# vwxyzjn/cleanrl

Measured on NVIDIA H100. Metric: env steps/sec (SPS) PPO Breakout num_envs=1024, higher is better.
Workload: dtype bf16

## Files before the change

cleanrl_b200/csrc/net_tc.cu:

```cuda
#include <cuda.h>
#include <algorithm>
#include "tc_base.cuh"
#include "tc_conv_win.cuh"
#include "tc_conv1_u8.cuh"
#include "tc_gemm_tma.cuh"
#include "tc_wgrad_win.cuh"
#include "tc_reduce.cuh"
#include "tc_aux.cuh"
#include "tc_heads.cuh"
#include "tc_heads_wide.cuh"
#include "tc_lstm.cuh"

namespace b200rl {

struct NatureLayout {
    int A;
    int64_t c1w, c1b, c2w, c2b, c3w, c3b, fcw, fcb, hw, hb, total;
    int64_t w1f, w2f, w2dg, w3f, w3dg, wfcf, wfcdg, w1l, w1sc, packed_total;
    bool wide; int G; int64_t whf, whdg, hbp;
    int64_t wih, whh, bih, bhh, whhp;
    explicit NatureLayout(int A_) : A(A_), wih(-1), whh(-1), bih(-1), bhh(-1), whhp(-1) {
        int64_t o = 0;
        c1w = o; o += 32 * 4 * 8 * 8;  c1b = o; o += 32;
        c2w = o; o += 64 * 32 * 4 * 4; c2b = o; o += 64;
// ... 76 lines not shown
    }
};

static void gemm_rowmajor(KGemmParams& p, const bf16* x, int64_t n, int nchunks) {
    memset(&p, 0, sizeof(p));
    p.scale = 1.f;
    p.A = x; p.M = n; p.nchunks = nchunks;
}


static void win_defaults(WinParams& p) { memset(&p, 0, sizeof(p)); p.scale = 1.f; }
static int round8(int v) { return (v + 7) & ~7; }
static void win_conv1(WinParams& p, const bf16* x0, const int64_t* rows, int64_t n) {
    p.A = x0; p.rows = rows; p.n = (int)n; p.G = 441; p.Wp = 21; p.M = n * 441;
    p.tpi_shift = 2;
    p.n_images = rows ? (int64_t)1 << 24 : n;
    p.ntaps = 4; p.shift[0] = 0; p.shift[1] = 1; p.shift[2] = 21; p.shift[3] = 22; p.WR = round8(128 + 22);
}
static void win_conv2(WinParams& p, const bf16* act1, int64_t n) {
    p.A = act1; p.n = (int)n; p.G = 100; p.Wp = 10; p.M = n * 100;
    p.ntaps = 4; p.shift[0] = 0; p.shift[1] = 1; p.shift[2] = 10; p.shift[3] = 11; p.WR = round8(128 + 11);
}
static void win_conv3(WinParams& p, const bf16* act2, int64_t n) {
    p.A = act2; p.n = (int)n; p.G = 81; p.Wp = 9; p.M = n * 81;
    p.ntaps = 9; for (int ky = 0; ky < 3; ++ky) for (int kx = 0; kx < 3; ++kx) p.shift[ky * 3 + kx] = ky * 9 + kx;
    p.WR = round8(128 + 20);
}
static void wgw_defaults(WGradWinParams& w) { memset(&w, 0, sizeof(w)); }

static const int kC1Ctas = 264, kC2Ctas = 132, kC3Ctas = 132;
static WPlan conv1_wgrad_plan(int64_t n, bool u8) {
    return u8 ? wgrad_plan(n * 512, kC2Ctas, 512) : wgrad_plan(n * 512, kC1Ctas, 128);
}
static WPlan conv2_wgrad_plan(int64_t n) { return wgrad_plan(n * 100, kC2Ctas, 128); }
static WPlan conv3_wgrad_plan(int64_t n) { return wgrad_plan(n * 81, kC3Ctas, 128); }

static size_t wgrad_win_bytes(int splits, int nslots) { return (size_t)splits * nslots * 64 * 64 * sizeof(float); }
static size_t wgrad_win_bias_bytes(int splits) { return (size_t)splits * 64 * sizeof(float); }
static int launch_wgrad_win(const WGradWinParams& p, int ctas, cudaStream_t s, const char* what) {
    const size_t smem = (size_t)kWgradWinStages * ((size_t)p.WRX * 128 * p.cpr + 128 * 128) + 4096 + 1024;
    static SmemAttrCache attr;
    if (int rc0 = attr.ensure(tc_wgrad_win, smem, what)) return rc0;
    CUtensorMap tmX, tmY;
    memset(&tmX, 0, sizeof(tmX)); memset(&tmY, 0, sizeof(tmY));
    const int use_tma = p.tpi_shift ? 0 : 1;
    if (p.rows_per_cta % 128 != 0) return fail(B200RL_ERR_INVALID_ARGUMENT, "%s: rows per CTA must be a multiple of 128", what);
    if (ctas < 1 || (int64_t)(ctas - 1) * p.rows_per_cta >= p.M)
        return fail(B200RL_ERR_INVALID_ARGUMENT, "%s: every row split must own at least one row", what);
    int rc;
    if (use_tma) {
        if (p.rows || p.ldy != 64 || p.ncolsY != 64)
            return fail(B200RL_ERR_INVALID_ARGUMENT, "%s: linear-grid mode needs contiguous rows and 64-channel dY", what);
        if ((rc = make_tmap_2d(&tmX, p.X, p.M, (int64_t)p.cpr * 64, p.WRX, what))) return rc;
        if ((rc = make_tmap_2d(&tmY, p.Y, p.M, 64, 128, what))) return rc;
    } else {
        if ((128 << p.tpi_shift) < p.G) return fail(B200RL_ERR_INVALID_ARGUMENT, "%s: steps per image too small", what);
        if ((rc = make_tmap_3d(&tmX, p.X, p.n_images, p.G, (int64_t)p.cpr * 64, p.WRX, what))) return rc;
    }
    const dim3 grid((unsigned)ceil_div(p.nslots / 2, kWgradWinTilesPerCta), ctas);
    tc_wgrad_win<<<grid, kWgradWinThreads, smem, s>>>(tmX, tmY, p, use_tma);
    return check_launch(what);
}

}

using namespace b200rl;

namespace b200rl {
static bool head_ok(int A) { return A >= 1 && A < kMaxWideHeads; }
static size_t wide_dhead_bytes(int64_t n, const NatureLayout& L) { return ((size_t)n * L.G * 2 + 255) & ~(size_t)255; }
static size_t wide_small_bytes(int64_t n, const NatureLayout& L, int A1) {
    return wide_dhead_bytes(n, L) + colsum_f32_ws(n, A1);
}

static int trunk_fwd(const NatureLayout& L, const NatureActs& Q, const float* params, const bf16* P, bf16* act, int64_t n,
                     cudaStream_t s) {
    int rc;
    KGemmParams p;
    WinParams wp;
    win_defaults(wp); win_conv2(wp, act + Q.act1, n);
    wp.Bw = P + L.w2f; wp.N = 64; wp.vH = 9; wp.vW = 9; wp.out_mode = WOUT_DENSE; wp.out = act + Q.act2;
    wp.bias = params + L.c2b; wp.relu = 1; wp.mask_out = reinterpret_cast<uint32_t*>(act + Q.m2);
    { ProfScope ps(s, "conv2_fwd", 2.0 * n * 81 * 64 * 512, (double)n * ((12800 + 5184) * 2 + 648));
      if ((rc = launch_conv_win_t<128, 2, 2, 4>(wp, s, "naturecnn/conv2"))) return rc; }
    win_defaults(wp); win_conv3(wp, act + Q.act2, n);
    wp.Bw = P + L.w3f; wp.N = 64; wp.vH = 7; wp.vW = 7; wp.out_mode = WOUT_DENSE; wp.out = act + Q.act3;
    wp.bias = params + L.c3b; wp.relu = 1; wp.mask_out = reinterpret_cast<uint32_t*>(act + Q.m3);
    { ProfScope ps(s, "conv3_fwd", 2.0 * n * 49 * 64 * 576, (double)n * ((5184 + 3136) * 2 + 392));
      if ((rc = launch_conv_win_t<128, 1, 4, 9>(wp, s, "naturecnn/conv3"))) return rc; }
    gemm_rowmajor(p, act + Q.act3, n, 49);
    p.Bw = P + L.wfcf; p.N = 512; p.out = act + Q.hid; p.ldo = 512; p.bias = params + L.fcb; p.relu = 1;
    p.mask_out = reinterpret_cast<uint32_t*>(act + Q.m4);
    { ProfScope ps(s, "fc_fwd", 2.0 * n * 512 * 3136, (double)n * (3136 + 512) * 2 + 512.0 * 3136 * 2);
      if (n <= 8192) { if ((rc = launch_gemm_tma<64, 6>(p, s, "naturecnn/fc"))) return rc; }
      else if ((rc = launch_gemm_tma<128, 3>(p, s, "naturecnn/fc"))) return rc; }
    return B200RL_OK;
}

static int trunk_bwd(const NatureLayout& L, const NatureActs& Q, const bf16* P, bf16* act, float* grads, int64_t n,
                     float* wsbig, float* wssmall, void* tail_ready_event, bool dact1_fused, cudaStream_t s) {
    int rc;
    KGemmParams p;
    {
        int splits;
        { ProfScope ps(s, "fc_wgrad", 2.0 * n * 512 * 3136, (double)n * (3136 + 512) * 2 + 512.0 * 3136 * 4);
          if ((splits = launch_wgrad_tma(act + Q.dhid, 512, act + Q.act3, 3136, n, wsbig, s, "naturecnn/fc_wgrad")) < 0) return splits; }
        { ProfScope ps(s, "wgrad_fold_bias", 0, 0);
          note_launches(1); tc_fold_fc<<<(unsigned)ceil_div((int64_t)512 * 3136, 256), 256, 0, s>>>(wsbig, splits, 512, 13 * 256, 512, 3136, 64, 49, 1.f, grads + L.fcw);
          if ((rc = colsum(act + Q.dhid, n, 512, 512, wssmall, grads + L.fcb, s))) return rc; }
        if (tail_ready_event) {
            cudaError_t e = cudaEventRecord(reinterpret_cast<cudaEvent_t>(tail_ready_event), s);
            if (e != cudaSuccess) return fail(B200RL_ERR_CUDA, "naturecnn_backward: cudaEventRecord: %s", cudaGetErrorString(e));
        }
        gemm_rowmajor(p, act + Q.dhid, n, 8);
        p.Bw = P + L.wfcdg; p.N = 3136; p.out = act + Q.dact3a; p.out2 = act + Q.dact3b; p.dual_dact3 = 1;
        p.ldo = 3136; p.mask_bits = reinterpret_cast<const uint32_t*>(act + Q.m3);
        { ProfScope ps(s, "fc_dgrad", 2.0 * n * 512 * 3136, (double)n * ((3136 + 512) * 2 + 392) + 512.0 * 3136 * 2);
          if ((rc = launch_gemm_tma<128, 3>(p, s, "naturecnn/fc_dgrad"))) return rc; }
    }
    WGradWinParams gw;
    WinParams wp;
    FoldWin fw;
    {
        wgw_defaults(gw);
        gw.X = act + Q.act2; gw.M = n * 81; gw.n = (int)n; gw.G = 81; gw.cpr = 1; gw.nslots = 10; gw.WRX = round8(128 + 20);
        for (int t = 0; t < 9; ++t) gw.shift[t] = (t / 3) * 9 + (t % 3);
        const int st[10] = {0, 1, 2, 3, 4, 5, 6, 7, 7, 8};
        for (int k = 0; k < 10; ++k) { gw.slot_tap[k] = st[k]; gw.slot_cc[k] = 0; }
        gw.Y = act + Q.dact3a; gw.ldy = 64; gw.ncolsY = 64;
        const WPlan pl = conv3_wgrad_plan(n);
        gw.rows_per_cta = pl.rows_per_cta; gw.ws = wsbig; gw.wsb = wssmall;
        { ProfScope ps(s, "conv3_wgrad", 2.0 * n * 49 * 64 * 576, (double)n * (5184 + 5184) * 2);
          if ((rc = launch_wgrad_win(gw, pl.splits, s, "naturecnn/conv3_wgrad"))) return rc; }
        memset(&fw, 0, sizeof(fw));
        fw.layer = 3; fw.S = pl.splits; fw.nslots = 10; fw.Cout = 64; fw.scale = 1.f; fw.bscale = 1.f;
        for (int k = 0; k < 10; ++k) { fw.slot_tap[k] = st[k]; fw.slot_skip[k] = (k == 8); }
        { ProfScope ps(s, "wgrad_fold_bias", 0, 0);
          fw.wsb = wssmall; fw.db = grads + L.c3b;
          tc_fold_win<<<(unsigned)ceil_div(640 * 64 + 64, 32), 256, 0, s>>>(wsbig, fw, grads + L.c3w);
          if ((rc = check_launch("naturecnn/conv3_fold"))) return rc; }
        win_defaults(wp);
        wp.A = act + Q.dact3b; wp.n = (int)n; wp.G = 121; wp.Wp = 11; wp.M = n * 121; wp.ntaps = 9;
        for (int ky = 0; ky < 3; ++ky) for (int kx = 0; kx < 3; ++kx) wp.shift[ky * 3 + kx] = (2 - ky) * 11 + (2 - kx);
        wp.WR = round8(128 + 24);
        wp.Bw = P + L.w3dg; wp.N = 64; wp.vH = 9; wp.vW = 9; wp.out_mode = WOUT_DACT2;
        wp.out = act + Q.dact2a; wp.out2 = act + Q.dact2b; wp.mask_bits = reinterpret_cast<const uint32_t*>(act + Q.m2);
        { ProfScope ps(s, "conv3_dgrad", 2.0 * n * 81 * 64 * 576, (double)n * ((7744 + 6400 + 7744) * 2 + 648));
          if ((rc = launch_conv_win_t<128, 1, 4, 9>(wp, s, "naturecnn/conv3_dgrad"))) return rc; }
    }
    {
        wgw_defaults(gw);
        gw.X = act + Q.act1; gw.M = n * 100; gw.n = (int)n; gw.G = 100; gw.cpr = 2; gw.nslots = 8; gw.WRX = round8(128 + 11);
        gw.shift[0] = 0; gw.shift[1] = 1; gw.shift[2] = 10; gw.shift[3] = 11;
        for (int k = 0; k < 8; ++k) { gw.slot_tap[k] = k >> 1; gw.slot_cc[k] = k & 1; }
        gw.Y = act + Q.dact2a; gw.ldy = 64; gw.ncolsY = 64;
        const WPlan pl = conv2_wgrad_plan(n);
        gw.rows_per_cta = pl.rows_per_cta; gw.ws = wsbig; gw.wsb = wssmall;
        { ProfScope ps(s, "conv2_wgrad", 2.0 * n * 81 * 64 * 512, (double)n * (12800 + 6400) * 2);
          if ((rc = launch_wgrad_win(gw, pl.splits, s, "naturecnn/conv2_wgrad"))) return rc; }
        memset(&fw, 0, sizeof(fw));
        fw.layer = 2; fw.S = pl.splits; fw.nslots = 8; fw.Cout = 64; fw.scale = 1.f; fw.bscale = 1.f;
        for (int k = 0; k < 8; ++k) { fw.slot_tap[k] = k >> 1; fw.slot_cc[k] = k & 1; }
        { ProfScope ps(s, "wgrad_fold_bias", 0, 0);
          fw.wsb = wssmall; fw.db = grads + L.c2b;
          tc_fold_win<<<(unsigned)ceil_div(512 * 64 + 64, 32), 256, 0, s>>>(wsbig, fw, grads + L.c2w);
          if ((rc = check_launch("naturecnn/conv2_fold"))) return rc; }
        if (dact1_fused) return B200RL_OK;
        win_defaults(wp);
        wp.A = act + Q.dact2b; wp.n = (int)n; wp.G = 121; wp.Wp = 11; wp.M = n * 121; wp.ntaps = 4;
        for (int a = 0; a < 2; ++a) for (int b = 0; b < 2; ++b) wp.shift[a * 2 + b] = (1 - a) * 11 + (1 - b);
        wp.WR = round8(128 + 12);
        wp.Bw = P + L.w2dg; wp.N = 128; wp.vH = 10; wp.vW = 10; wp.out_mode = WOUT_DACT1;
        wp.out = act + Q.dact1; wp.mask_bits = reinterpret_cast<const uint32_t*>(act + Q.m1);
        { ProfScope ps(s, "conv2_dgrad", 2.0 * n * 400 * 32 * 256, (double)n * ((7744 + 14112) * 2 + 1600));
          if ((rc = launch_conv_win<128, 1, 4, 4>(wp, s, "naturecnn/conv2_dgrad"))) return rc; }
    }
    return B200RL_OK;
}
static size_t trunk_big_bytes(int64_t n) {
    return std::max({wgrad_tma_bytes(n, 512, 3136), wgrad_win_bytes(conv3_wgrad_plan(n).splits, 10),
                     wgrad_win_bytes(conv2_wgrad_plan(n).splits, 8)});
}
static size_t trunk_small_bytes(int64_t n) {
    return std::max({colsum_ws(n, 512), wgrad_win_bias_bytes(conv3_wgrad_plan(n).splits),
                     wgrad_win_bias_bytes(conv2_wgrad_plan(n).splits)});
}

static int wide_head_fwd(const NatureLayout& L, const bf16* P, const bf16* hid, int64_t n, int A1, float* out, cudaStream_t s) {
    KGemmParams p;
    gemm_rowmajor(p, hid, n, 8);
    p.Bw = P + L.whf; p.N = L.G; p.bias = reinterpret_cast<const float*>(P + L.hbp);
    p.out_f32 = out; p.ldo = A1; p.ncols_f32 = A1;
    return launch_gemm_tma<128, 3>(p, s, "wide_heads");
}

static int wide_head_bwd(const NatureLayout& L, const bf16* P, const float* dhead, int64_t n, int A1, const bf16* hid, bf16* dhid,
                         const uint32_t* hid_bits, float* dW, float* db, float* wsbig, float* wssmall, cudaStream_t s) {
    int rc;
    KGemmParams p;
    bf16* dh16 = reinterpret_cast<bf16*>(wssmall);
    float* dbpart = reinterpret_cast<float*>(reinterpret_cast<char*>(wssmall) + wide_dhead_bytes(n, L));
    int cb = (int)ceil_div(n * L.G, 256); if (cb > num_sms() * 8) cb = num_sms() * 8;
    tc_head_dhead_bf16<<<cb, 256, 0, s>>>(dhead, n, A1, L.G, dh16);
    if ((rc = check_launch("wide_heads_dhead"))) return rc;
    if ((rc = colsum_f32(dhead, n, A1, dbpart, db, s))) return rc;
    const int splits = launch_wgrad_tma(dh16, L.G, hid, 512, n, wsbig, s, "wide_heads_wgrad");
    if (splits < 0) return splits;
    tc_fold_fc<<<(unsigned)ceil_div((int64_t)A1 * 512, 256), 256, 0, s>>>(wsbig, splits, L.G, 512, A1, 512, 512, 1, 1.f, dW);
    if ((rc = check_launch("wide_heads_wgrad"))) return rc;
    gemm_rowmajor(p, dh16, n, L.G / 64);
    p.Bw = P + L.whdg; p.N = 512; p.out = dhid; p.ldo = 512;
    p.mask_bits = hid_bits;
    if (n <= 8192) { if ((rc = launch_gemm_tma<64, 6>(p, s, "wide_heads_dgrad"))) return rc; }
    else if ((rc = launch_gemm_tma<128, 3>(p, s, "wide_heads_dgrad"))) return rc;
    return B200RL_OK;
}
}

extern "C" int64_t b200rl_naturecnn_param_count(int A) { return A >= 1 ? NatureLayout(A).total : -1; }
extern "C" int64_t b200rl_naturecnn_grad_tail_offset(int A) { return A >= 1 ? NatureLayout(A).fcw : -1; }
extern "C" size_t b200rl_naturecnn_bf16_packed_bytes(int A) { return head_ok(A) ? (size_t)NatureLayout(A).packed_total * 2 : 0; }
extern "C" size_t b200rl_naturecnn_bf16_acts_bytes(int64_t n, int obs_format) {
    return n >= 0 ? (size_t)NatureActs(n, obs_format == B200RL_OBS_U8_NCHW).total * 2 + 256 : 0;
}

extern "C" int b200rl_frames_to_s2d_bf16(const uint8_t* obs, const int64_t* rows, int64_t n, void* out, void* stream) {
    B200RL_REQUIRE(n >= 0, "frames_to_s2d: negative n");
    if (n == 0) return B200RL_OK;
    B200RL_REQUIRE(obs && out, "frames_to_s2d: null pointer");
    B200RL_REQUIRE(aligned(obs, 4) && aligned(out, 16), "frames_to_s2d: misaligned buffer");
    cudaStream_t s = (cudaStream_t)stream;
// ... 373 lines not shown
```

cleanrl_b200/csrc/tc_conv_win.cuh:

```cuda
#pragma once
#include "tc_base.cuh"

namespace b200rl {
using namespace tc;

enum { WOUT_DENSE = 0, WOUT_S2D2 = 1, WOUT_DACT2 = 2, WOUT_DACT1 = 3 };
struct WinParams {
    const bf16* A;
    const int64_t* rows;
    int64_t M;
    int n, G, Wp;
    int tpi_shift;
    int64_t n_images;
    int ntaps;
    int shift[16];
    int WR;
    const bf16* Bw;
    int N;
    int vH, vW;
    int out_mode;
    bf16* out;
    bf16* out2;
    const uint32_t* mask_bits;
    uint32_t* mask_out;
// ... 168 lines not shown
                        const float f = __uint_as_float(v[e]);
                        bits |= (f > 0.f ? 1u : 0u) << e;
                    }
                    if (p.mask_out) p.mask_out[ob + g] = bits;
                }
                if (p.mask_bits) {
#pragma unroll
                    for (int e = 0; e < 32; ++e) if (!((mb[g] >> e) & 1u)) v[e] = 0u;
                }
                int4 w[4];
                if (p.relu) {
#pragma unroll
                    for (int e = 0; e < 4; ++e) {
                        w[e].x = (int)pack_bf16x2_relu(__uint_as_float(v[8 * e]), __uint_as_float(v[8 * e + 1]));
                        w[e].y = (int)pack_bf16x2_relu(__uint_as_float(v[8 * e + 2]), __uint_as_float(v[8 * e + 3]));
                        w[e].z = (int)pack_bf16x2_relu(__uint_as_float(v[8 * e + 4]), __uint_as_float(v[8 * e + 5]));
                        w[e].w = (int)pack_bf16x2_relu(__uint_as_float(v[8 * e + 6]), __uint_as_float(v[8 * e + 7]));
                    }
                } else {
#pragma unroll
                for (int e = 0; e < 4; ++e) {
                    w[e].x = (int)pack_bf16x2(__uint_as_float(v[8 * e]), __uint_as_float(v[8 * e + 1]));
                    w[e].y = (int)pack_bf16x2(__uint_as_float(v[8 * e + 2]), __uint_as_float(v[8 * e + 3]));
                    w[e].z = (int)pack_bf16x2(__uint_as_float(v[8 * e + 4]), __uint_as_float(v[8 * e + 5]));
                    w[e].w = (int)pack_bf16x2(__uint_as_float(v[8 * e + 6]), __uint_as_float(v[8 * e + 7]));
                }
                }
                if (p.out_mode == WOUT_DACT1) {
                    int4* brow = reinterpret_cast<int4*>(st + lr * LDA) + 8 * g + 4 * (g & 1);
#pragma unroll
                    for (int e = 0; e < 4; ++e) brow[e] = w[e];
                } else {
                    bf16* dst = p.out + o1 + g * 32;
                    st_global_32b(dst, w[0], w[1]);
                    st_global_32b(dst + 16, w[2], w[3]);
                }
            }
            if (p.out_mode == WOUT_DACT1) {
                if (half == 0)
                    *reinterpret_cast<int64_t*>(st + lr * LDA + BN) = valid ? ((int64_t)i * 441 + 2 * Y * 21 + 2 * X) * 32 : -1;
                named_bar(1 + wg, 128);
#pragma unroll
                for (int m = 0; m < 8; ++m) {
                    const int k = m * 128 + wt, g = (k >> 2) & 3, e = k & 3;
                    const float* srow = st + (k >> 4) * LDA;
                    const int64_t o = *reinterpret_cast<const int64_t*>(srow + BN);
                    if (o < 0) continue;
                    const int4 val = reinterpret_cast<const int4*>(srow)[8 * g + 4 * (g & 1) + e];
                    *reinterpret_cast<int4*>(p.out + o + (g >> 1) * 21 * 32 + (g & 1) * 32 + e * 8) = val;
                }
            }
        }
    }
}

template <int BN, int CPR, int STAGES, int NTAPS>
static int launch_conv_win(const WinParams& p, cudaStream_t s, const char* what) {
    if (p.ntaps != NTAPS) return fail(B200RL_ERR_INVALID_ARGUMENT, "%s: %d taps, kernel instance has %d", what, p.ntaps, NTAPS);
    if (p.out_mode != WOUT_S2D2 && p.out_mode != WOUT_DACT1)
        return fail(B200RL_ERR_INVALID_ARGUMENT, "%s: dense and conv3 data-gradient outputs run on tc_conv_win_t", what);
    if (p.out_mode == WOUT_DACT1 && (BN != 128 || p.N != 128))
        return fail(B200RL_ERR_INVALID_ARGUMENT, "%s: the conv2 data gradient stores 4 groups of 32 channels per cell", what);
    const size_t smem = (size_t)p.ntaps * CPR * BN * 128 + (size_t)STAGES * p.WR * 128 * CPR + conv_win_acc_bytes<BN>() + 1024;
    static SmemAttrCache attr;
    if (int rc = attr.ensure(tc_conv_win<BN, CPR, STAGES, NTAPS>, smem, what)) return rc;
    if ((int64_t)p.G * p.Wp >= 65536 || p.G < 1 || p.N % 32 != 0)
        return fail(B200RL_ERR_INVALID_ARGUMENT, "%s: grid %d x width %d outside the epilogue's multiply-shift range, or N %% 32 != 0", what, p.G, p.Wp);
    if (p.rows && !p.tpi_shift) return fail(B200RL_ERR_INVALID_ARGUMENT, "%s: the image gather needs image-aligned tiling", what);
    if (p.tpi_shift && (128 << p.tpi_shift) < p.G) return fail(B200RL_ERR_INVALID_ARGUMENT, "%s: tiles per image too small", what);
    const int total = p.tpi_shift ? (int)((int64_t)p.n << p.tpi_shift) : (int)ceil_div(p.M, 128);
    int grid = num_sms();
    if (grid > total) grid = total;
    CUtensorMap tmA;
    memset(&tmA, 0, sizeof(tmA));
    int rc;
    if (p.tpi_shift) rc = make_tmap_3d(&tmA, p.A, p.n_images, p.G, (int64_t)CPR * 64, p.WR, what);
    else rc = make_tmap_2d(&tmA, p.A, p.M, (int64_t)CPR * 64, p.WR, what);
    if (rc) return rc;
    tc_conv_win<BN, CPR, STAGES, NTAPS><<<grid, kConvWinThreads, smem, s>>>(tmA, p, total);
    return check_launch(what);
}

constexpr int kConvWinTThreads = 384;
constexpr int kConvWinTLds = 64 + 4;
template <int BP>
__host__ __device__ constexpr size_t conv_win_t_stage_bytes() { return (size_t)2 * BP * kConvWinTLds * sizeof(float); }

template <int R>
__device__ __forceinline__ void stage_acc_transposed(float* st, int wg_tid, const float (&d)[R]) {
    const int co = ((wg_tid >> 5) << 4) + ((wg_tid & 31) >> 2), pos = (wg_tid & 3) * 2;
#pragma unroll
    for (int j = 0; j < R / 4; ++j) {
        float* p0 = st + (8 * j + pos) * kConvWinTLds + co;
        p0[0] = d[4 * j];
        p0[kConvWinTLds] = d[4 * j + 1];
        p0[8] = d[4 * j + 2];
        p0[kConvWinTLds + 8] = d[4 * j + 3];
    }
}

template <int BP, int CPR, int STAGES, int NTAPS>
__global__ void __launch_bounds__(kConvWinTThreads, 1) tc_conv_win_t(const __grid_constant__ CUtensorMap tmA, const WinParams p,
                                                                     int total_tiles) {
    static_assert(BP % 128 == 0, "one thread per position row of a 128-row slice");
    static_assert(STAGES % 2 == 0, "each consumer warpgroup owns every other stage");
    constexpr int RPT = BP / 128;
    constexpr int A_CHUNK = 64 * 128;
    constexpr int LDS = kConvWinTLds;
    extern __shared__ uint8_t smem_raw[];
    __shared__ uint64_t full_bar[STAGES], empty_bar[STAGES];
    uint8_t* smem = reinterpret_cast<uint8_t*>((reinterpret_cast<uintptr_t>(smem_raw) + 1023) & ~uintptr_t(1023));
    const int tid = threadIdx.x, warp = tid >> 5;
    const int nchunks = NTAPS * CPR;
    const int K = nchunks * 64;
    const int IMG = p.WR * 128;
    const int STAGE_BYTES = IMG * CPR;
    uint8_t* sW = smem;
    uint8_t* sRing = smem + (size_t)nchunks * A_CHUNK;
    float* sAcc = reinterpret_cast<float*>(sRing + (size_t)STAGES * STAGE_BYTES);

    if (tid == 0) {
        for (int s = 0; s < STAGES; ++s) { mbar_init(&full_bar[s], 1); mbar_init(&empty_bar[s], 4); }
        fence_barrier_init();
        tma_prefetch_desc(&tmA);
    }
    for (int idx = tid; idx < nchunks * 64 * 8; idx += blockDim.x) {
        const int c16 = idx & 7;
        const int t = idx >> 3;
        const int r = t & 63, j = t >> 6;
        int4 v = make_int4(0, 0, 0, 0);
        if (r < p.N) v = ldg16(p.Bw + (int64_t)r * K + j * 64 + c16 * 8);
        *reinterpret_cast<int4*>(sW + (size_t)j * A_CHUNK + img_off(r, c16)) = v;
    }
    fence_proxy_async_smem();
    __syncthreads();
    const int tile_begin = (int)(((int64_t)total_tiles * blockIdx.x) / gridDim.x);
    const int tile_end = (int)(((int64_t)total_tiles * (blockIdx.x + 1)) / gridDim.x);

    if (warp == 0) {
        if (tid == 0) {
            uint32_t q = 0;
            for (int tile = tile_begin; tile < tile_end; ++tile, ++q) {
                const uint32_t s = q % STAGES;
                if (q >= (uint32_t)STAGES) mbar_wait(&empty_bar[s], ((q / STAGES) - 1) & 1);
                const uint32_t dst = smem_u32(sRing + (size_t)s * STAGE_BYTES);
                mbar_arrive_expect_tx(&full_bar[s], (uint32_t)STAGE_BYTES);
#pragma unroll
                for (int c = 0; c < CPR; ++c) tma_load_2d(dst + c * IMG, &tmA, c * 64, tile * BP, &full_bar[s]);
            }
        }
    } else if (warp >= 4) {
        const int wg = (warp - 4) >> 2, wt = tid & 127;
        float* st = sAcc + wg * BP * LDS;
        const uint32_t w_base = smem_u32(sW);
        const uint32_t mW = (65536u + (uint32_t)p.Wp - 1u) / (uint32_t)p.Wp;
        constexpr int NW = 2;
        float d[BP / 2];
#pragma unroll
        for (int e = 0; e < BP / 2; ++e) d[e] = 0.f;
        for (int tile = tile_begin + wg; tile < tile_end; tile += 2) {
            const uint32_t q = (uint32_t)(tile - tile_begin), s = q % STAGES;
            mbar_wait(&full_bar[s], (q / STAGES) & 1);
            wgmma_fence();
            const uint32_t win = smem_u32(sRing + (size_t)s * STAGE_BYTES);
#pragma unroll
            for (int t = 0; t < NTAPS; ++t) {
#pragma unroll
                for (int c = 0; c < CPR; ++c) {
                    const uint64_t b = desc_kmajor(win + (uint32_t)(c * IMG) + (uint32_t)p.shift[t] * 128u);
                    const uint64_t a = desc_kmajor(w_base + (uint32_t)((t * CPR + c) * A_CHUNK));
#pragma unroll
                    for (int kk = 0; kk < 4; ++kk)
                        WgmmaBf16<BP, 0, 0>::mma(d, a + 2 * kk, b + 2 * kk, (t | c | kk) != 0 ? 1u : 0u);
                }
            }
            wgmma_commit();
            bool valid[RPT];
            int64_t o1[RPT], o2[RPT], ob[RPT];
            uint32_t mb[RPT][NW];
#pragma unroll
            for (int rr = 0; rr < RPT; ++rr) {
                const int64_t r = (int64_t)tile * BP + rr * 128 + wt;
                const int i = (int)(r / p.G);
                const int rem = (int)(r - (int64_t)i * p.G);
                const int Y = (int)(((uint32_t)rem * mW) >> 16), X = rem - Y * p.Wp;
                valid[rr] = r < p.M && (Y < p.vH) && (X < p.vW);
                o2[rr] = 0;
                if (p.out_mode == WOUT_DENSE) {
                    const int64_t orow = ((int64_t)i * p.vH + Y) * p.vW + X;
                    o1[rr] = orow * p.N; ob[rr] = orow * (p.N >> 5);
                } else {
                    o1[rr] = ((int64_t)i * 100 + Y * 10 + X) * 64;
                    o2[rr] = ((int64_t)i * 121 + (Y + 1) * 11 + (X + 1)) * 64;
                    ob[rr] = ((int64_t)i * 81 + Y * 9 + X) * 2;
                }
                mb[rr][0] = mb[rr][1] = 0xFFFFFFFFu;
                if (p.mask_bits != nullptr && valid[rr]) {
                    const uint2 t = __ldg(reinterpret_cast<const uint2*>(p.mask_bits + ob[rr]));
                    mb[rr][0] = t.x; mb[rr][1] = t.y;
                }
            }
            wgmma_wait<0>();
            wgmma_fence_operands(d);
            if ((tid & 31) == 0) mbar_arrive(&empty_bar[s]);
            named_bar(1 + wg, 128);
            stage_acc_transposed(st, wt, d);
            named_bar(1 + wg, 128);
#pragma unroll
            for (int rr = 0; rr < RPT; ++rr) {
                float* srow = st + (rr * 128 + wt) * LDS;
#pragma unroll
                for (int g = 0; g < NW; ++g) {
                    if (!valid[rr] || g * 32 >= p.N) continue;
                    uint32_t v[32];
#pragma unroll
                    for (int e = 0; e < 8; ++e) {
                        const float4 f = *reinterpret_cast<const float4*>(srow + g * 32 + 4 * e);
                        v[4 * e] = __float_as_uint(f.x); v[4 * e + 1] = __float_as_uint(f.y);
                        v[4 * e + 2] = __float_as_uint(f.z); v[4 * e + 3] = __float_as_uint(f.w);
                    }
                    if (p.bias) {
                        const float4* bp = reinterpret_cast<const float4*>(p.bias + g * 32);
#pragma unroll
                        for (int e = 0; e < 8; ++e) {
                            const float4 bv = __ldg(bp + e);
                            v[4 * e] = __float_as_uint(fmaf(__uint_as_float(v[4 * e]), p.scale, bv.x));
                            v[4 * e + 1] = __float_as_uint(fmaf(__uint_as_float(v[4 * e + 1]), p.scale, bv.y));
                            v[4 * e + 2] = __float_as_uint(fmaf(__uint_as_float(v[4 * e + 2]), p.scale, bv.z));
                            v[4 * e + 3] = __float_as_uint(fmaf(__uint_as_float(v[4 * e + 3]), p.scale, bv.w));
                        }
                    } else {
#pragma unroll
                        for (int e = 0; e < 32; ++e) v[e] = __float_as_uint(__uint_as_float(v[e]) * p.scale);
                    }
                    if (p.relu) {
                        uint32_t bits = 0u;
#pragma unroll
                        for (int e = 0; e < 32; ++e) bits |= (__uint_as_float(v[e]) > 0.f ? 1u : 0u) << e;
                        if (p.mask_out) p.mask_out[ob[rr] + g] = bits;
                    }
                    if (p.mask_bits) {
#pragma unroll
                        for (int e = 0; e < 32; ++e) if (!((mb[rr][g] >> e) & 1u)) v[e] = 0u;
                    }
                    int4 w[4];
                    if (p.relu) {
#pragma unroll
                        for (int e = 0; e < 4; ++e) {
                            w[e].x = (int)pack_bf16x2_relu(__uint_as_float(v[8 * e]), __uint_as_float(v[8 * e + 1]));
                            w[e].y = (int)pack_bf16x2_relu(__uint_as_float(v[8 * e + 2]), __uint_as_float(v[8 * e + 3]));
                            w[e].z = (int)pack_bf16x2_relu(__uint_as_float(v[8 * e + 4]), __uint_as_float(v[8 * e + 5]));
                            w[e].w = (int)pack_bf16x2_relu(__uint_as_float(v[8 * e + 6]), __uint_as_float(v[8 * e + 7]));
                        }
                    } else {
#pragma unroll
                        for (int e = 0; e < 4; ++e) {
                            w[e].x = (int)pack_bf16x2(__uint_as_float(v[8 * e]), __uint_as_float(v[8 * e + 1]));
                            w[e].y = (int)pack_bf16x2(__uint_as_float(v[8 * e + 2]), __uint_as_float(v[8 * e + 3]));
                            w[e].z = (int)pack_bf16x2(__uint_as_float(v[8 * e + 4]), __uint_as_float(v[8 * e + 5]));
                            w[e].w = (int)pack_bf16x2(__uint_as_float(v[8 * e + 6]), __uint_as_float(v[8 * e + 7]));
                        }
                    }
                    int4* brow = reinterpret_cast<int4*>(srow) + 4 * g;
#pragma unroll
                    for (int e = 0; e < 4; ++e) brow[e] = w[e];
                }
                *reinterpret_cast<longlong2*>(srow + 64) = make_longlong2(valid[rr] ? o1[rr] : -1, o2[rr]);
            }
            named_bar(1 + wg, 128);
#pragma unroll
            for (int m = 0; m < BP / 16; ++m) {
                const int k = m * 128 + wt, part = k & 7;
                const float* srow = st + (k >> 3) * LDS;
                const longlong2 off = *reinterpret_cast<const longlong2*>(srow + 64);
                if (off.x < 0) continue;
                const int4 val = reinterpret_cast<const int4*>(srow)[part];
                *reinterpret_cast<int4*>(p.out + off.x + part * 8) = val;
                if (p.out_mode == WOUT_DACT2) *reinterpret_cast<int4*>(p.out2 + off.y + part * 8) = val;
            }
        }
    }
}

template <int BP, int CPR, int STAGES, int NTAPS>
static int launch_conv_win_t(WinParams p, cudaStream_t s, const char* what) {
    if (p.ntaps != NTAPS) return fail(B200RL_ERR_INVALID_ARGUMENT, "%s: %d taps, kernel instance has %d", what, p.ntaps, NTAPS);
    if (p.N != 64) return fail(B200RL_ERR_INVALID_ARGUMENT, "%s: N = %d, the kernel computes 64 output channels", what, p.N);
    if ((int64_t)p.G * p.Wp >= 65536 || p.G < 1)
        return fail(B200RL_ERR_INVALID_ARGUMENT, "%s: grid %d x width %d outside the epilogue's multiply-shift range", what, p.G, p.Wp);
    if (p.rows || p.tpi_shift) return fail(B200RL_ERR_INVALID_ARGUMENT, "%s: the channel-major kernel walks a contiguous linear grid", what);
    if (p.out_mode != WOUT_DENSE && p.out_mode != WOUT_DACT2)
        return fail(B200RL_ERR_INVALID_ARGUMENT, "%s: only bf16 dense and conv3 data-gradient outputs in this kernel", what);
    int maxs = 0;
    for (int t = 0; t < NTAPS; ++t) maxs = p.shift[t] > maxs ? p.shift[t] : maxs;
    p.WR = (BP + maxs + 7) & ~7;
    if (p.WR > 256) return fail(B200RL_ERR_INVALID_ARGUMENT, "%s: window of %d rows exceeds a TMA box", what, p.WR);
    const size_t smem = (size_t)NTAPS * CPR * 64 * 128 + (size_t)STAGES * p.WR * 128 * CPR + conv_win_t_stage_bytes<BP>() + 1024;
    static SmemAttrCache attr;
    if (int rc = attr.ensure(tc_conv_win_t<BP, CPR, STAGES, NTAPS>, smem, what)) return rc;
    const int total = (int)ceil_div(p.M, BP);
    int grid = num_sms();
    if (grid > total) grid = total;
    CUtensorMap tmA;
    memset(&tmA, 0, sizeof(tmA));
    if (int rc = make_tmap_2d(&tmA, p.A, p.M, (int64_t)CPR * 64, p.WR, what)) return rc;
    tc_conv_win_t<BP, CPR, STAGES, NTAPS><<<grid, kConvWinTThreads, smem, s>>>(tmA, p, total);
    return check_launch(what);
}

}
```

Before: 1.256 million.

## Rework conv window epilogue with stmatrix bf16 staging, TMA weight load, ordered warpgroups

```diff
diff --git a/cleanrl_b200/csrc/net_tc.cu b/cleanrl_b200/csrc/net_tc.cu
--- a/cleanrl_b200/csrc/net_tc.cu
+++ b/cleanrl_b200/csrc/net_tc.cu
@@ -182,12 +182,12 @@
     wp.Bw = P + L.w2f; wp.N = 64; wp.vH = 9; wp.vW = 9; wp.out_mode = WOUT_DENSE; wp.out = act + Q.act2;
     wp.bias = params + L.c2b; wp.relu = 1; wp.mask_out = reinterpret_cast<uint32_t*>(act + Q.m2);
     { ProfScope ps(s, "conv2_fwd", 2.0 * n * 81 * 64 * 512, (double)n * ((12800 + 5184) * 2 + 648));
-      if ((rc = launch_conv_win_t<128, 2, 2, 4>(wp, s, "naturecnn/conv2"))) return rc; }
+      if ((rc = launch_conv_win_t<128, 2, 3, 4>(wp, s, "naturecnn/conv2"))) return rc; }
     win_defaults(wp); win_conv3(wp, act + Q.act2, n);
     wp.Bw = P + L.w3f; wp.N = 64; wp.vH = 7; wp.vW = 7; wp.out_mode = WOUT_DENSE; wp.out = act + Q.act3;
     wp.bias = params + L.c3b; wp.relu = 1; wp.mask_out = reinterpret_cast<uint32_t*>(act + Q.m3);
     { ProfScope ps(s, "conv3_fwd", 2.0 * n * 49 * 64 * 576, (double)n * ((5184 + 3136) * 2 + 392));
-      if ((rc = launch_conv_win_t<128, 1, 4, 9>(wp, s, "naturecnn/conv3"))) return rc; }
+      if ((rc = launch_conv_win_t<128, 1, 6, 9>(wp, s, "naturecnn/conv3"))) return rc; }
     gemm_rowmajor(p, act + Q.act3, n, 49);
     p.Bw = P + L.wfcf; p.N = 512; p.out = act + Q.hid; p.ldo = 512; p.bias = params + L.fcb; p.relu = 1;
     p.mask_out = reinterpret_cast<uint32_t*>(act + Q.m4);
@@ -246,7 +246,7 @@
         wp.Bw = P + L.w3dg; wp.N = 64; wp.vH = 9; wp.vW = 9; wp.out_mode = WOUT_DACT2;
         wp.out = act + Q.dact2a; wp.out2 = act + Q.dact2b; wp.mask_bits = reinterpret_cast<const uint32_t*>(act + Q.m2);
         { ProfScope ps(s, "conv3_dgrad", 2.0 * n * 81 * 64 * 576, (double)n * ((7744 + 6400 + 7744) * 2 + 648));
-          if ((rc = launch_conv_win_t<128, 1, 4, 9>(wp, s, "naturecnn/conv3_dgrad"))) return rc; }
+          if ((rc = launch_conv_win_t<128, 1, 6, 9>(wp, s, "naturecnn/conv3_dgrad"))) return rc; }
     }
     {
         wgw_defaults(gw);
diff --git a/cleanrl_b200/csrc/tc_conv_win.cuh b/cleanrl_b200/csrc/tc_conv_win.cuh
--- a/cleanrl_b200/csrc/tc_conv_win.cuh
+++ b/cleanrl_b200/csrc/tc_conv_win.cuh
@@ -274,63 +274,63 @@
 }
 
 constexpr int kConvWinTThreads = 384;
-constexpr int kConvWinTLds = 64 + 4;
+constexpr int kConvWinTRow = 128 + 16;
 template <int BP>
-__host__ __device__ constexpr size_t conv_win_t_stage_bytes() { return (size_t)2 * BP * kConvWinTLds * sizeof(float); }
-
-template <int R>
-__device__ __forceinline__ void stage_acc_transposed(float* st, int wg_tid, const float (&d)[R]) {
-    const int co = ((wg_tid >> 5) << 4) + ((wg_tid & 31) >> 2), pos = (wg_tid & 3) * 2;
-#pragma unroll
-    for (int j = 0; j < R / 4; ++j) {
-        float* p0 = st + (8 * j + pos) * kConvWinTLds + co;
-        p0[0] = d[4 * j];
-        p0[kConvWinTLds] = d[4 * j + 1];
-        p0[8] = d[4 * j + 2];
-        p0[kConvWinTLds + 8] = d[4 * j + 3];
-    }
+__host__ __device__ constexpr size_t conv_win_t_stage_bytes() {
+    return (size_t)2 * BP * (kConvWinTRow + 2 * sizeof(uint32_t));
+}
+
+__device__ __forceinline__ uint32_t gather_nibble_bits(uint32_t x) {
+    x &= 0x11111111u;
+    x = (x | (x >> 3)) & 0x03030303u;
+    x = (x | (x >> 6)) & 0x000F000Fu;
+    return (x | (x >> 12)) & 0xFFu;
+}
+
+__device__ __forceinline__ void named_bar_arrive(int id, int n) { asm volatile("bar.arrive %0, %1;" ::"r"(id), "r"(n) : "memory"); }
+
+__device__ __forceinline__ void stmatrix_x4_trans(uint32_t addr, uint32_t r0, uint32_t r1, uint32_t r2, uint32_t r3) {
+    asm volatile("stmatrix.sync.aligned.m8n8.x4.trans.shared.b16 [%0], {%1, %2, %3, %4};"
+                 ::"r"(addr), "r"(r0), "r"(r1), "r"(r2), "r"(r3) : "memory");
 }
 
 template <int BP, int CPR, int STAGES, int NTAPS>
-__global__ void __launch_bounds__(kConvWinTThreads, 1) tc_conv_win_t(const __grid_constant__ CUtensorMap tmA, const WinParams p,
+__global__ void __launch_bounds__(kConvWinTThreads, 1) tc_conv_win_t(const __grid_constant__ CUtensorMap tmA,
+                                                                     const __grid_constant__ CUtensorMap tmW, const WinParams p,
                                                                      int total_tiles) {
     static_assert(BP % 128 == 0, "one thread per position row of a 128-row slice");
-    static_assert(STAGES % 2 == 0, "each consumer warpgroup owns every other stage");
+    static_assert(BP % 16 == 0, "stmatrix stores two 8-position blocks at a time");
     constexpr int RPT = BP / 128;
     constexpr int A_CHUNK = 64 * 128;
-    constexpr int LDS = kConvWinTLds;
+    constexpr int ROW = kConvWinTRow;
     extern __shared__ uint8_t smem_raw[];
-    __shared__ uint64_t full_bar[STAGES], empty_bar[STAGES];
+    __shared__ uint64_t full_bar[STAGES], empty_bar[STAGES], w_bar;
     uint8_t* smem = reinterpret_cast<uint8_t*>((reinterpret_cast<uintptr_t>(smem_raw) + 1023) & ~uintptr_t(1023));
     const int tid = threadIdx.x, warp = tid >> 5;
-    const int nchunks = NTAPS * CPR;
-    const int K = nchunks * 64;
+    constexpr int nchunks = NTAPS * CPR;
     const int IMG = p.WR * 128;
     const int STAGE_BYTES = IMG * CPR;
     uint8_t* sW = smem;
     uint8_t* sRing = smem + (size_t)nchunks * A_CHUNK;
-    float* sAcc = reinterpret_cast<float*>(sRing + (size_t)STAGES * STAGE_BYTES);
+    uint8_t* sRows = sRing + (size_t)STAGES * STAGE_BYTES;
+    uint32_t* sBits = reinterpret_cast<uint32_t*>(sRows + (size_t)2 * BP * ROW);
 
     if (tid == 0) {
         for (int s = 0; s < STAGES; ++s) { mbar_init(&full_bar[s], 1); mbar_init(&empty_bar[s], 4); }
+        mbar_init(&w_bar, 1);
         fence_barrier_init();
         tma_prefetch_desc(&tmA);
+        tma_prefetch_desc(&tmW);
     }
-    for (int idx = tid; idx < nchunks * 64 * 8; idx += blockDim.x) {
-        const int c16 = idx & 7;
-        const int t = idx >> 3;
-        const int r = t & 63, j = t >> 6;
-        int4 v = make_int4(0, 0, 0, 0);
-        if (r < p.N) v = ldg16(p.Bw + (int64_t)r * K + j * 64 + c16 * 8);
-        *reinterpret_cast<int4*>(sW + (size_t)j * A_CHUNK + img_off(r, c16)) = v;
-    }
-    fence_proxy_async_smem();
     __syncthreads();
     const int tile_begin = (int)(((int64_t)total_tiles * blockIdx.x) / gridDim.x);
     const int tile_end = (int)(((int64_t)total_tiles * (blockIdx.x + 1)) / gridDim.x);
 
     if (warp == 0) {
         if (tid == 0) {
+            mbar_arrive_expect_tx(&w_bar, (uint32_t)(nchunks * A_CHUNK));
+#pragma unroll
+            for (int j = 0; j < nchunks; ++j) tma_load_2d(smem_u32(sW + (size_t)j * A_CHUNK), &tmW, j * 64, 0, &w_bar);
             uint32_t q = 0;
             for (int tile = tile_begin; tile < tile_end; ++tile, ++q) {
                 const uint32_t s = q % STAGES;
@@ -342,17 +342,26 @@
             }
         }
     } else if (warp >= 4) {
-        const int wg = (warp - 4) >> 2, wt = tid & 127;
-        float* st = sAcc + wg * BP * LDS;
+        const int wg = (warp - 4) >> 2, wt = tid & 127, lane = tid & 31, wq = wt >> 5;
+        uint8_t* st = sRows + (size_t)wg * BP * ROW;
+        uint32_t* sb = sBits + wg * 2 * BP;
         const uint32_t w_base = smem_u32(sW);
         const uint32_t mW = (65536u + (uint32_t)p.Wp - 1u) / (uint32_t)p.Wp;
-        constexpr int NW = 2;
+        const int co = wq * 16 + (lane >> 2), g = wq >> 1, cb = co & 31;
+        const float scale = p.scale;
+        const float bias_lo = p.bias ? __ldg(p.bias + co) : 0.f, bias_hi = p.bias ? __ldg(p.bias + co + 8) : 0.f;
+        const bool want_bits = p.relu && p.mask_out != nullptr;
+        const uint32_t st_addr = smem_u32(st) + (uint32_t)((((lane >> 4) << 3) + (lane & 7)) * ROW + wq * 32 + ((lane >> 3) & 1) * 16);
         float d[BP / 2];
 #pragma unroll
         for (int e = 0; e < BP / 2; ++e) d[e] = 0.f;
+        const int ntiles = tile_end - tile_begin;
+        const bool ordered = p.out_mode == WOUT_DENSE;
+        mbar_wait(&w_bar, 0);
         for (int tile = tile_begin + wg; tile < tile_end; tile += 2) {
             const uint32_t q = (uint32_t)(tile - tile_begin), s = q % STAGES;
             mbar_wait(&full_bar[s], (q / STAGES) & 1);
+            if (ordered && q > 0) named_bar(3 + wg, 256);
             wgmma_fence();
             const uint32_t win = smem_u32(sRing + (size_t)s * STAGE_BYTES);
 #pragma unroll
@@ -368,107 +377,100 @@
             }
             wgmma_commit();
             bool valid[RPT];
-            int64_t o1[RPT], o2[RPT], ob[RPT];
-            uint32_t mb[RPT][NW];
+            int64_t ob[RPT];
+            longlong2 off[RPT];
+            uint2 mb[RPT];
 #pragma unroll
             for (int rr = 0; rr < RPT; ++rr) {
-                const int64_t r = (int64_t)tile * BP + rr * 128 + wt;
-                const int i = (int)(r / p.G);
-                const int rem = (int)(r - (int64_t)i * p.G);
+                const int r = tile * BP + rr * 128 + wt;
+                const int i = (int)((uint32_t)r / (uint32_t)p.G);
+                const int rem = r - i * p.G;
                 const int Y = (int)(((uint32_t)rem * mW) >> 16), X = rem - Y * p.Wp;
                 valid[rr] = r < p.M && (Y < p.vH) && (X < p.vW);
-                o2[rr] = 0;
+                int64_t o1, o2 = 0;
                 if (p.out_mode == WOUT_DENSE) {
                     const int64_t orow = ((int64_t)i * p.vH + Y) * p.vW + X;
-                    o1[rr] = orow * p.N; ob[rr] = orow * (p.N >> 5);
+                    o1 = orow * p.N; ob[rr] = orow * (p.N >> 5);
                 } else {
-                    o1[rr] = ((int64_t)i * 100 + Y * 10 + X) * 64;
-                    o2[rr] = ((int64_t)i * 121 + (Y + 1) * 11 + (X + 1)) * 64;
+                    o1 = ((int64_t)i * 100 + Y * 10 + X) * 64;
+                    o2 = ((int64_t)i * 121 + (Y + 1) * 11 + (X + 1)) * 64;
                     ob[rr] = ((int64_t)i * 81 + Y * 9 + X) * 2;
                 }
-                mb[rr][0] = mb[rr][1] = 0xFFFFFFFFu;
-                if (p.mask_bits != nullptr && valid[rr]) {
-                    const uint2 t = __ldg(reinterpret_cast<const uint2*>(p.mask_bits + ob[rr]));
-                    mb[rr][0] = t.x; mb[rr][1] = t.y;
-                }
+                off[rr] = make_longlong2(valid[rr] ? o1 : -1, o2);
+                mb[rr] = make_uint2(0xFFFFFFFFu, 0xFFFFFFFFu);
+                if (p.mask_bits != nullptr && valid[rr]) mb[rr] = __ldg(reinterpret_cast<const uint2*>(p.mask_bits + ob[rr]));
+            }
+            named_bar(1 + wg, 128);
+#pragma unroll
+            for (int rr = 0; rr < RPT; ++rr) {
+                const int pos = rr * 128 + wt;
+                *reinterpret_cast<longlong2*>(st + pos * ROW + 128) = off[rr];
+                if (p.mask_bits) { sb[pos] = mb[rr].x; sb[BP + pos] = mb[rr].y; }
             }
             wgmma_wait<0>();
             wgmma_fence_operands(d);
-            if ((tid & 31) == 0) mbar_arrive(&empty_bar[s]);
-            named_bar(1 + wg, 128);
-            stage_acc_transposed(st, wt, d);
-            named_bar(1 + wg, 128);
-#pragma unroll
-            for (int rr = 0; rr < RPT; ++rr) {
-                float* srow = st + (rr * 128 + wt) * LDS;
-#pragma unroll
-                for (int g = 0; g < NW; ++g) {
-                    if (!valid[rr] || g * 32 >= p.N) continue;
-                    uint32_t v[32];
-#pragma unroll
-                    for (int e = 0; e < 8; ++e) {
-                        const float4 f = *reinterpret_cast<const float4*>(srow + g * 32 + 4 * e);
-                        v[4 * e] = __float_as_uint(f.x); v[4 * e + 1] = __float_as_uint(f.y);
-                        v[4 * e + 2] = __float_as_uint(f.z); v[4 * e + 3] = __float_as_uint(f.w);
+            if (lane == 0) mbar_arrive(&empty_bar[s]);
+            if (ordered && (int)q + 1 < ntiles) named_bar_arrive(3 + (wg ^ 1), 256);
+            if (p.mask_bits) named_bar(1 + wg, 128);
+            uint32_t bl[BP / 32], bh[BP / 32];
+#pragma unroll
+            for (int t = 0; t < BP / 32; ++t) bl[t] = bh[t] = 0u;
+#pragma unroll
+            for (int jp = 0; jp < BP / 16; ++jp) {
+                uint32_t pk[4];
+#pragma unroll
+                for (int u = 0; u < 2; ++u) {
+                    const int j = 2 * jp + u;
+                    float v[4];
+                    if (p.bias) {
+#pragma unroll
+                        for (int e = 0; e < 4; ++e) v[e] = fmaf(d[4 * j + e], scale, e < 2 ? bias_lo : bias_hi);
+                    } else {
+#pragma unroll
+                        for (int e = 0; e < 4; ++e) v[e] = d[4 * j + e] * scale;
                     }
-                    if (p.bias) {
-                        const float4* bp = reinterpret_cast<const float4*>(p.bias + g * 32);
-#pragma unroll
-                        for (int e = 0; e < 8; ++e) {
-                            const float4 bv = __ldg(bp + e);
-                            v[4 * e] = __float_as_uint(fmaf(__uint_as_float(v[4 * e]), p.scale, bv.x));
-                            v[4 * e + 1] = __float_as_uint(fmaf(__uint_as_float(v[4 * e + 1]), p.scale, bv.y));
-                            v[4 * e + 2] = __float_as_uint(fmaf(__uint_as_float(v[4 * e + 2]), p.scale, bv.z));
-                            v[4 * e + 3] = __float_as_uint(fmaf(__uint_as_float(v[4 * e + 3]), p.scale, bv.w));
+                    if (want_bits) {
+                        const uint32_t l0 = __ballot_sync(0xFFFFFFFFu, v[0] > 0.f), l1 = __ballot_sync(0xFFFFFFFFu, v[1] > 0.f);
+                        const uint32_t h0 = __ballot_sync(0xFFFFFFFFu, v[2] > 0.f), h1 = __ballot_sync(0xFFFFFFFFu, v[3] > 0.f);
+                        if ((j & 3) == (lane >> 3)) {
+                            bl[j >> 2] = (lane & 1) ? l1 : l0;
+                            bh[j >> 2] = (lane & 1) ? h1 : h0;
                         }
-                    } else {
-#pragma unroll
-                        for (int e = 0; e < 32; ++e) v[e] = __float_as_uint(__uint_as_float(v[e]) * p.scale);
-                    }
-                    if (p.relu) {
-                        uint32_t bits = 0u;
-#pragma unroll
-                        for (int e = 0; e < 32; ++e) bits |= (__uint_as_float(v[e]) > 0.f ? 1u : 0u) << e;
-                        if (p.mask_out) p.mask_out[ob[rr] + g] = bits;
                     }
                     if (p.mask_bits) {
-#pragma unroll
-                        for (int e = 0; e < 32; ++e) if (!((mb[rr][g] >> e) & 1u)) v[e] = 0u;
+                        const uint2 w = *reinterpret_cast<const uint2*>(sb + g * BP + 8 * j + 2 * (lane & 3));
+                        if (!((w.x >> cb) & 1u)) v[0] = 0.f;
+                        if (!((w.y >> cb) & 1u)) v[1] = 0.f;
+                        if (!((w.x >> (cb + 8)) & 1u)) v[2] = 0.f;
+                        if (!((w.y >> (cb + 8)) & 1u)) v[3] = 0.f;
                     }
-                    int4 w[4];
-                    if (p.relu) {
-#pragma unroll
-                        for (int e = 0; e < 4; ++e) {
-                            w[e].x = (int)pack_bf16x2_relu(__uint_as_float(v[8 * e]), __uint_as_float(v[8 * e + 1]));
-                            w[e].y = (int)pack_bf16x2_relu(__uint_as_float(v[8 * e + 2]), __uint_as_float(v[8 * e + 3]));
-                            w[e].z = (int)pack_bf16x2_relu(__uint_as_float(v[8 * e + 4]), __uint_as_float(v[8 * e + 5]));
-                            w[e].w = (int)pack_bf16x2_relu(__uint_as_float(v[8 * e + 6]), __uint_as_float(v[8 * e + 7]));
-                        }
-                    } else {
-#pragma unroll
-                        for (int e = 0; e < 4; ++e) {
-                            w[e].x = (int)pack_bf16x2(__uint_as_float(v[8 * e]), __uint_as_float(v[8 * e + 1]));
-                            w[e].y = (int)pack_bf16x2(__uint_as_float(v[8 * e + 2]), __uint_as_float(v[8 * e + 3]));
-                            w[e].z = (int)pack_bf16x2(__uint_as_float(v[8 * e + 4]), __uint_as_float(v[8 * e + 5]));
-                            w[e].w = (int)pack_bf16x2(__uint_as_float(v[8 * e + 6]), __uint_as_float(v[8 * e + 7]));
-                        }
-                    }
-                    int4* brow = reinterpret_cast<int4*>(srow) + 4 * g;
-#pragma unroll
-                    for (int e = 0; e < 4; ++e) brow[e] = w[e];
-                }
-                *reinterpret_cast<longlong2*>(srow + 64) = make_longlong2(valid[rr] ? o1[rr] : -1, o2[rr]);
+                    pk[2 * u] = p.relu ? pack_bf16x2_relu(v[0], v[1]) : pack_bf16x2(v[0], v[1]);
+                    pk[2 * u + 1] = p.relu ? pack_bf16x2_relu(v[2], v[3]) : pack_bf16x2(v[2], v[3]);
+                }
+                stmatrix_x4_trans(st_addr + (uint32_t)(16 * jp * ROW), pk[0], pk[1], pk[2], pk[3]);
+            }
+            if (want_bits) {
+                uint16_t* sb16 = reinterpret_cast<uint16_t*>(sb);
+                const int qp = (lane & 7) >> 1;
+#pragma unroll
+                for (int t = 0; t < BP / 32; ++t)
+                    sb16[(32 * t + lane) * 4 + wq] = (uint16_t)(gather_nibble_bits(bl[t] >> qp) | (gather_nibble_bits(bh[t] >> qp) << 8));
             }
             named_bar(1 + wg, 128);
+            if (want_bits) {
+#pragma unroll
+                for (int rr = 0; rr < RPT; ++rr)
+                    if (valid[rr]) *reinterpret_cast<uint2*>(p.mask_out + ob[rr]) = *reinterpret_cast<const uint2*>(sb + 2 * (rr * 128 + wt));
+            }
 #pragma unroll
             for (int m = 0; m < BP / 16; ++m) {
                 const int k = m * 128 + wt, part = k & 7;
-                const float* srow = st + (k >> 3) * LDS;
-                const longlong2 off = *reinterpret_cast<const longlong2*>(srow + 64);
-                if (off.x < 0) continue;
+                const uint8_t* srow = st + (k >> 3) * ROW;
+                const longlong2 o = *reinterpret_cast<const longlong2*>(srow + 128);
+                if (o.x < 0) continue;
                 const int4 val = reinterpret_cast<const int4*>(srow)[part];
-                *reinterpret_cast<int4*>(p.out + off.x + part * 8) = val;
-                if (p.out_mode == WOUT_DACT2) *reinterpret_cast<int4*>(p.out2 + off.y + part * 8) = val;
+                *reinterpret_cast<int4*>(p.out + o.x + part * 8) = val;
+                if (p.out_mode == WOUT_DACT2) *reinterpret_cast<int4*>(p.out2 + o.y + part * 8) = val;
             }
         }
     }
@@ -481,6 +483,8 @@
     if ((int64_t)p.G * p.Wp >= 65536 || p.G < 1)
         return fail(B200RL_ERR_INVALID_ARGUMENT, "%s: grid %d x width %d outside the epilogue's multiply-shift range", what, p.G, p.Wp);
     if (p.rows || p.tpi_shift) return fail(B200RL_ERR_INVALID_ARGUMENT, "%s: the channel-major kernel walks a contiguous linear grid", what);
+    if (p.M < 1 || p.M > (int64_t)INT32_MAX - BP)
+        return fail(B200RL_ERR_INVALID_ARGUMENT, "%s: %lld grid positions outside the epilogue's 32-bit position range", what, (long long)p.M);
     if (p.out_mode != WOUT_DENSE && p.out_mode != WOUT_DACT2)
         return fail(B200RL_ERR_INVALID_ARGUMENT, "%s: only bf16 dense and conv3 data-gradient outputs in this kernel", what);
     int maxs = 0;
@@ -493,10 +497,12 @@
     const int total = (int)ceil_div(p.M, BP);
     int grid = num_sms();
     if (grid > total) grid = total;
-    CUtensorMap tmA;
+    CUtensorMap tmA, tmW;
     memset(&tmA, 0, sizeof(tmA));
+    memset(&tmW, 0, sizeof(tmW));
     if (int rc = make_tmap_2d(&tmA, p.A, p.M, (int64_t)CPR * 64, p.WR, what)) return rc;
-    tc_conv_win_t<BP, CPR, STAGES, NTAPS><<<grid, kConvWinTThreads, smem, s>>>(tmA, p, total);
+    if (int rc = make_tmap_2d(&tmW, p.Bw, 64, (int64_t)NTAPS * CPR * 64, 64, what)) return rc;
+    tc_conv_win_t<BP, CPR, STAGES, NTAPS><<<grid, kConvWinTThreads, smem, s>>>(tmA, tmW, p, total);
     return check_launch(what);
 }
 
```

Result: faster. 1.295 million, median of 6 (+3.1%).
